# SavaRobotics/FoundationPose

Measured on AMD Instinct MI355X. Metric: pose-hypotheses/sec (render+refine+score), 252 hyp x 160x160, higher is better.
Workload: dtype f16

## Files before the change

foundationpose_amd/csrc/attn.hip:

```cpp
#include "common.h"
#include "device_util.h"
#include "pose_math.h"

#define AT_DH 128
#define AT_TP 416
#define AT_MAXT 400
#define FA_WAVES 7
#define FA_NSTAGE 3
#define FA_AHEAD 2
#define FA_DMA_PER_WAVE 5
#define FA_THREADS (FA_WAVES * 64)
#define FA_QB (FA_WAVES * 32)
#define FA_KB 64
#define FA_STAGE_HALFS (FA_KB * AT_DH * 2)
#define FA_QW_HALFS (32 * AT_DH)
#define FA_LDS_BYTES ((FA_NSTAGE * FA_STAGE_HALFS + FA_WAVES * FA_QW_HALFS) * 2)


typedef float f32x2 __attribute__((ext_vector_type(2)));
template <bool V> struct FaBool { static constexpr bool value = V; };

#ifdef HALO_STAMP
__device__ unsigned long long g_attn_stamps[1024 * 7 * 32];
extern "C" __attribute__((visibility("default"))) int fp_dbg_attn_stamps(unsigned long long *host) {
  return hipMemcpyFromSymbol(host, HIP_SYMBOL(g_attn_stamps), sizeof(g_attn_stamps)) == hipSuccess ? 0 : -1;
}
#define ASTAMP(i) do { if (blockIdx.x < 1024 && stamp_on) st[(i)] = __builtin_amdgcn_s_memtime(); } while (0)
#else
#define ASTAMP(i) do { } while (0)
#endif

__device__ __forceinline__ float fa_max3(float a, float b, float c) {
  float r;
  asm("v_max3_f32 %0, %1, %2, %3" : "=v"(r) : "v"(a), "v"(b), "v"(c));
  return r;
}

__global__ __launch_bounds__(FA_THREADS, 2) void attention_kernel(const f16 *__restrict__ qk, const f16 *__restrict__ vt, int T,
                                                                  f16 *__restrict__ out, int n_items) {
  extern __shared__ __attribute__((aligned(16))) f16 smem[];
  const int nqb = (T + FA_QB - 1) / FA_QB;
  const int tid = threadIdx.x, lane = tid & 63, wave = __builtin_amdgcn_readfirstlane(tid >> 6);
  const int lr = lane & 31, lh = lane >> 5;
  const int nkb = (T + FA_KB - 1) / FA_KB;
  const int G = gridDim.x;
  f16 *qlds = smem + FA_NSTAGE * FA_STAGE_HALFS + wave * FA_QW_HALFS;
#ifdef HALO_STAMP
  unsigned long long st[32];
#pragma unroll
  for (int i = 0; i < 32; ++i) st[i] = 0;
  bool stamp_on = true;
#endif
  ASTAMP(0);

  auto item_of = [&](int v, int &b, int &h, int &qb) __attribute__((always_inline)) {
    const int L = xcd_remap(v, n_items);
    qb = L % nqb;
    h = (L / nqb) & 3;
    b = L / (nqb * 4);
  };

  unsigned sx[FA_DMA_PER_WAVE], sadd[FA_DMA_PER_WAVE];
#pragma unroll
  for (int u = 0; u < FA_DMA_PER_WAVE; ++u) {
    int i = wave + u * FA_WAVES;
    if (i >= 32) i -= 32;
    if (i < 16) {
      const int c = i * 64 + lane, kl = c >> 4, chp = c & 15;
      sx[u] = kl;
      sadd[u] = ((chp ^ (kl & 15)) * 8) * 2;
    } else {
      const int c = (i - 16) * 64 + lane, d = c >> 3, chp = c & 7;
      sx[u] = (chp ^ ((d >> 1) & 7)) * 8;
      sadd[u] = d * AT_TP * 2;
    }
  }
  int s_v = blockIdx.x, s_kb = 0, s_slot = 0;
  const f16 *s_kbase, *s_vsrc;
  auto stage_bases = [&]() __attribute__((always_inline)) {
    int b, h, qb;
    item_of(s_v, b, h, qb);
    s_kbase = qk + (size_t)b * T * 1024 + 512 + h * AT_DH;
    s_vsrc = vt + ((size_t)b * 4 + h) * AT_DH * AT_TP;
  };
  stage_bases();
  auto stage_next = [&]() __attribute__((always_inline)) {
#pragma unroll
    for (int u = 0; u < FA_DMA_PER_WAVE; ++u) {
      int i = wave + u * FA_WAVES;
      if (i >= 32) i -= 32;
      const bool is_k = i < 16;
      const unsigned t = min((unsigned)(s_kb * FA_KB) + sx[u], is_k ? (unsigned)(T - 1) : 408u);
      const unsigned voff = t * (is_k ? 2048u : 2u) + sadd[u];
      glds16(is_k ? s_kbase : s_vsrc, voff, smem + s_slot * FA_STAGE_HALFS + i * 512);
    }
    s_slot = s_slot + 1 == FA_NSTAGE ? 0 : s_slot + 1;
    if (++s_kb == nkb) {
      s_kb = 0;
      s_v += G;
      if (s_v < n_items) stage_bases();
    }
  };
  const unsigned qrow = wave * 32 + lr;
  auto stage_q = [&](int v) __attribute__((always_inline)) {
    int b, h, qb;
    item_of(v, b, h, qb);
    const f16 *qbase = qk + ((size_t)b * T + qb * FA_QB) * 1024 + h * AT_DH;
    const unsigned voff = min(qrow, (unsigned)(T - 1 - qb * FA_QB)) * 2048u + lh * 16;
#pragma unroll
    for (int s = 0; s < 8; ++s) glds16(qbase + s * 16, voff, qlds + s * 512);
  };

  unsigned koffb[8], voffb[4];
#pragma unroll
  for (int s = 0; s < 8; ++s) koffb[s] = (lr * AT_DH + (((2 * s + lh) ^ (lr & 15)) * 8)) * 2;
#pragma unroll
  for (int s = 0; s < 4; ++s) voffb[s] = FA_KB * AT_DH * 2 + (lr * FA_KB + (((2 * s + lh) ^ ((lr >> 1) & 7)) * 8)) * 2;

  const float c2 = 0.08838834764831845f * 1.4426950408889634f;
  const f32x2 c2v = {c2, c2};

  int inflight = 0;
#pragma unroll
  for (int p = 0; p < FA_AHEAD; ++p)
    if (s_v < n_items) {
      stage_next();
      ++inflight;
    }
  stage_q((int)blockIdx.x);

  half8 qf[8];
  floatx16 oacc[4];
  float m_run, l_run;
  int c_slot = 0;
  int st_prev = 0;
  bool first = true;

  for (int v = blockIdx.x; v < n_items; v += G) {
    int b, h, qb;
    item_of(v, b, h, qb);
    const size_t rowbase = (size_t)b * T;
    const int q = qb * FA_QB + wave * 32 + lr;
    const bool wave_valid = qb * FA_QB + wave * 32 < T;
    const bool has_next = v + G < n_items;
#ifdef HALO_STAMP
    stamp_on = v == (int)blockIdx.x + G || n_items <= G;
#endif
    ASTAMP(1);
#pragma unroll
    for (int dt = 0; dt < 4; ++dt)
#pragma unroll
      for (int e = 0; e < 16; ++e) oacc[dt][e] = 0.f;
    m_run = -1.0e30f;
    l_run = 0.f;

    auto body = [&](const int kb, auto first_c, auto tail_c) __attribute__((always_inline)) {
      constexpr bool KB0 = decltype(first_c)::value;
      constexpr bool TAIL = decltype(tail_c)::value;
      int allowed = inflight > 1 ? 5 : 0;
      if (KB0) allowed = first ? 0 : (nkb == 1 ? st_prev : allowed + st_prev);
      else if (kb == 1 && has_next) allowed += 8;
      if (allowed == 0) wait_vm_lgkm<0>();
      else if (allowed == 5) wait_vm_lgkm<5>();
      else if (allowed == 8) wait_vm_lgkm<8>();
      else wait_vm_lgkm<13>();
      __builtin_amdgcn_s_barrier();
      __builtin_amdgcn_sched_barrier(0);
      ASTAMP(3 + 4 * kb);
      if (s_v < n_items) {
        stage_next();
        ++inflight;
      }
      if constexpr (KB0) {
#pragma unroll
        for (int s = 0; s < 8; ++s) qf[s] = *reinterpret_cast<const half8 *>(qlds + s * 512 + lane * 8);
      }
      const char *sb = reinterpret_cast<const char *>(smem) + c_slot * (FA_STAGE_HALFS * 2);
      floatx16 sacc[2];
#pragma unroll
      for (int sh = 0; sh < 2; ++sh) {
        half8 kf[2][4];
#pragma unroll
        for (int s = 0; s < 4; ++s)
#pragma unroll
          for (int kt = 0; kt < 2; ++kt) kf[kt][s] = *reinterpret_cast<const half8 *>(sb + koffb[sh * 4 + s] + kt * (32 * AT_DH * 2));
        __builtin_amdgcn_sched_barrier(0);
#pragma unroll
        for (int s = 0; s < 4; ++s)
#pragma unroll
          for (int kt = 0; kt < 2; ++kt) {
            if (sh == 0 && s == 0) {
              const floatx16 zero = {0.f, 0.f, 0.f, 0.f, 0.f, 0.f, 0.f, 0.f, 0.f, 0.f, 0.f, 0.f, 0.f, 0.f, 0.f, 0.f};
              sacc[kt] = __builtin_amdgcn_mfma_f32_32x32x16_f16(kf[kt][s], qf[0], zero, 0, 0, 0);
            } else {
              sacc[kt] = __builtin_amdgcn_mfma_f32_32x32x16_f16(kf[kt][s], qf[sh * 4 + s], sacc[kt], 0, 0, 0);
            }
          }
      }
      __builtin_amdgcn_sched_barrier(0);
      ASTAMP(4 + 4 * kb);
      if constexpr (KB0) {
        if (has_next) stage_q(v + G);
      }
      if constexpr (TAIL) {
#pragma unroll
        for (int kt = 0; kt < 2; ++kt)
#pragma unroll
          for (int r = 0; r < 16; ++r) {
            const int key = kb * FA_KB + kt * 32 + (r & 3) + 8 * (r >> 2) + 4 * lh;
            sacc[kt][r] = key < T ? sacc[kt][r] : -1.0e30f;
          }
      }
      float bm = fmaxf(sacc[0][15], sacc[1][15]);
      bm = fa_max3(bm, sacc[0][0], sacc[1][0]);
#pragma unroll
      for (int r = 1; r < 15; r += 2) bm = fa_max3(bm, sacc[0][r], sacc[0][r + 1]);
#pragma unroll
      for (int r = 1; r < 15; r += 2) bm = fa_max3(bm, sacc[1][r], sacc[1][r + 1]);
      bm = fmaxf(bm, __shfl_xor(bm, 32));
      const float m_new = fmaxf(m_run, bm);
      const float alpha = __builtin_amdgcn_exp2f((m_run - m_new) * c2);
      const float nmc = -m_new * c2;
      const f32x2 nmcv = {nmc, nmc};
      f32x2 ps2 = {0.f, 0.f};
#pragma unroll
      for (int kt = 0; kt < 2; ++kt)
#pragma unroll
        for (int r = 0; r < 16; r += 2) {
          const f32x2 sv = {sacc[kt][r], sacc[kt][r + 1]};
          const f32x2 ev = __builtin_elementwise_fma(sv, c2v, nmcv);
          const f32x2 e = {__builtin_amdgcn_exp2f(ev.x), __builtin_amdgcn_exp2f(ev.y)};
          sacc[kt][r] = e.x;
          sacc[kt][r + 1] = e.y;
          ps2 += e;
        }
      float ps = ps2.x + ps2.y;
      ps += __shfl_xor(ps, 32);
      l_run = l_run * alpha + ps;
      if (__builtin_amdgcn_ballot_w64(m_new != m_run) != 0) {
#pragma unroll
        for (int dt = 0; dt < 4; ++dt)
#pragma unroll
          for (int e = 0; e < 16; ++e) oacc[dt][e] *= alpha;
      }
      m_run = m_new;
      half8 pf[2][2];
#pragma unroll
      for (int kt = 0; kt < 2; ++kt)
#pragma unroll
        for (int s2 = 0; s2 < 2; ++s2)
#pragma unroll
          for (int j = 0; j < 8; ++j) pf[kt][s2][j] = (f16)sacc[kt][8 * s2 + j];
      __builtin_amdgcn_sched_barrier(0);
      ASTAMP(5 + 4 * kb);
#pragma unroll
      for (int kt = 0; kt < 2; ++kt) {
        half8 vf[2][4];
#pragma unroll
        for (int s2 = 0; s2 < 2; ++s2)
#pragma unroll
          for (int dt = 0; dt < 4; ++dt) vf[s2][dt] = *reinterpret_cast<const half8 *>(sb + voffb[kt * 2 + s2] + dt * (32 * FA_KB * 2));
        __builtin_amdgcn_sched_barrier(0);
#pragma unroll
        for (int s2 = 0; s2 < 2; ++s2)
#pragma unroll
          for (int dt = 0; dt < 4; ++dt) oacc[dt] = __builtin_amdgcn_mfma_f32_32x32x16_f16(vf[s2][dt], pf[kt][s2], oacc[dt], 0, 0, 0);
      }
      __builtin_amdgcn_sched_barrier(0);
      ASTAMP(6 + 4 * kb);
      c_slot = c_slot + 1 == FA_NSTAGE ? 0 : c_slot + 1;
      --inflight;
    };
    if (nkb == 1) {
      body(0, FaBool<true>{}, FaBool<true>{});
    } else {
      body(0, FaBool<true>{}, FaBool<false>{});
      for (int kb = 1; kb < nkb - 1; ++kb) body(kb, FaBool<false>{}, FaBool<false>{});
      body(nkb - 1, FaBool<false>{}, FaBool<true>{});
    }

    if (wave_valid) {
      const float inv = 1.f / l_run;
      f16 *orow = out + (rowbase + min(q, T - 1)) * 512 + h * AT_DH + lh * 8;
#pragma unroll
      for (int dt = 0; dt < 4; ++dt)
#pragma unroll
        for (int gq = 0; gq < 4; gq += 2) {
          half4 ha, hb;
#pragma unroll
          for (int j = 0; j < 4; ++j) ha[j] = (f16)(oacc[dt][gq * 4 + j] * inv), hb[j] = (f16)(oacc[dt][(gq + 1) * 4 + j] * inv);
          const uint2 ua = __builtin_bit_cast(uint2, ha), ub = __builtin_bit_cast(uint2, hb);
          const auto r0 = __builtin_amdgcn_permlane32_swap(ua.x, ub.x, false, false);
          const auto r1 = __builtin_amdgcn_permlane32_swap(ua.y, ub.y, false, false);
          const uint4 ov = {r0[0], r1[0], r0[1], r1[1]};
          if (q < T) *reinterpret_cast<uint4 *>(orow + dt * 32 + gq * 8) = ov;
        }
    }
    ASTAMP(2);
    st_prev = wave_valid ? 8 : 0;
    first = false;
  }
#ifdef HALO_STAMP
  if (blockIdx.x < 1024 && lane == 0) {
    st[31] = __builtin_amdgcn_s_memtime();
    unsigned long long *o = g_attn_stamps + ((size_t)blockIdx.x * 7 + wave) * 32;
#pragma unroll
    for (int i = 0; i < 32; ++i) o[i] = st[i];
  }
#endif
}

#define FS_WAVES 7
#define FS_KP 136
#define FS_VP 72
#define FS_AREA_BYTES (AT_DH * FS_VP * 2)
#define FS_LDS_BYTES (FS_WAVES * FS_AREA_BYTES + 2 * FS_WAVES * 32 * 4)
static_assert(64 * FS_KP * 2 <= FS_AREA_BYTES && AT_DH * 32 * 4 <= FS_AREA_BYTES, "attention_small: wave area");
__global__ __launch_bounds__(FS_WAVES * 64) void attention_small_kernel(const f16 *__restrict__ qk, const f16 *__restrict__ vt, int T, f16 *__restrict__ out) {
  extern __shared__ __attribute__((aligned(16))) char fs_lds[];
  float *fs_m = reinterpret_cast<float *>(fs_lds + FS_WAVES * FS_AREA_BYTES), *fs_l = fs_m + FS_WAVES * 32;
  const int tid = threadIdx.x, lane = tid & 63, w = __builtin_amdgcn_readfirstlane(tid >> 6), lr = lane & 31, lh = lane >> 5;
  const int nqt = (T + 31) >> 5, nkb = (T + 63) >> 6;
  const int qt = blockIdx.x % nqt, h = (blockIdx.x / nqt) & 3, b = blockIdx.x / (nqt * 4);
  const float c2 = 0.08838834764831845f * 1.4426950408889634f;
  f16 *area = reinterpret_cast<f16 *>(fs_lds + (size_t)w * FS_AREA_BYTES);
  if (w < nkb) {
    u32x4 kq[16], vq[16];
    {
      const f16 *kbase = qk + (size_t)b * T * 1024 + 512 + h * AT_DH;
#pragma unroll
      for (int u = 0; u < 16; ++u) {
        const int i = lane + 64 * u, key = min(w * 64 + (i >> 4), T - 1);
        kq[u] = *reinterpret_cast<const u32x4 *>(kbase + (size_t)key * 1024 + (i & 15) * 8);
      }
      const f16 *vbase = vt + ((size_t)b * 4 + h) * AT_DH * AT_TP;
#pragma unroll
      for (int u = 0; u < 16; ++u) {
        const int i = lane + 64 * u, col = min(w * 64 + (i & 7) * 8, 408);
        vq[u] = *reinterpret_cast<const u32x4 *>(vbase + (size_t)(i >> 3) * AT_TP + col);
      }
    }
    half8 qf[8];
    {
      const f16 *qrow = qk + ((size_t)b * T + min(qt * 32 + lr, T - 1)) * 1024 + h * AT_DH + lh * 8;
#pragma unroll
      for (int s = 0; s < 8; ++s) qf[s] = *reinterpret_cast<const half8 *>(qrow + s * 16);
    }
#pragma unroll
    for (int u = 0; u < 16; ++u) {
      const int i = lane + 64 * u;
      *reinterpret_cast<u32x4 *>(area + (i >> 4) * FS_KP + (i & 15) * 8) = kq[u];
    }
    wait_lgkm();
    half8 kf[2][8];
#pragma unroll
    for (int kt = 0; kt < 2; ++kt)
#pragma unroll
      for (int s = 0; s < 8; ++s) kf[kt][s] = *reinterpret_cast<const half8 *>(area + (kt * 32 + lr) * FS_KP + s * 16 + lh * 8);
    floatx16 sacc[2];
#pragma unroll
    for (int kt = 0; kt < 2; ++kt) {
#pragma unroll
      for (int e = 0; e < 16; ++e) sacc[kt][e] = 0.f;
#pragma unroll
      for (int s = 0; s < 8; ++s) sacc[kt] = __builtin_amdgcn_mfma_f32_32x32x16_f16(kf[kt][s], qf[s], sacc[kt], 0, 0, 0);
    }
#pragma unroll
    for (int kt = 0; kt < 2; ++kt)
#pragma unroll
      for (int r = 0; r < 16; ++r) {
        const int key = w * 64 + kt * 32 + (r & 3) + 8 * (r >> 2) + 4 * lh;
        sacc[kt][r] = key < T ? sacc[kt][r] : -1.0e30f;
      }
    float bm = fmaxf(sacc[0][0], sacc[1][0]);
#pragma unroll
    for (int r = 1; r < 16; ++r) bm = fmaxf(bm, fmaxf(sacc[0][r], sacc[1][r]));
    bm = fmaxf(bm, __shfl_xor(bm, 32));
    const float nmc = -bm * c2;
    float ps = 0.f;
#pragma unroll
    for (int kt = 0; kt < 2; ++kt)
#pragma unroll
      for (int r = 0; r < 16; ++r) {
        const float e = __builtin_amdgcn_exp2f(fmaf(sacc[kt][r], c2, nmc));
        sacc[kt][r] = e;
        ps += e;
      }
    ps += __shfl_xor(ps, 32);
    wait_lgkm();
#pragma unroll
    for (int u = 0; u < 16; ++u) {
      const int i = lane + 64 * u;
      *reinterpret_cast<u32x4 *>(area + (i >> 3) * FS_VP + (i & 7) * 8) = vq[u];
    }
    wait_lgkm();
    floatx16 oacc[4];
#pragma unroll
    for (int dt = 0; dt < 4; ++dt)
#pragma unroll
      for (int e = 0; e < 16; ++e) oacc[dt][e] = 0.f;
#pragma unroll
    for (int kt = 0; kt < 2; ++kt) {
      if (w * 64 + kt * 32 >= T) continue;
#pragma unroll
      for (int s2 = 0; s2 < 2; ++s2) {
        half8 pf;
#pragma unroll
        for (int j = 0; j < 8; ++j) pf[j] = (f16)sacc[kt][8 * s2 + j];
#pragma unroll
        for (int dt = 0; dt < 4; ++dt)
          oacc[dt] = __builtin_amdgcn_mfma_f32_32x32x16_f16(*reinterpret_cast<const half8 *>(area + (dt * 32 + lr) * FS_VP + kt * 32 + s2 * 16 + lh * 8), pf,
                                                            oacc[dt], 0, 0, 0);
      }
    }
    wait_lgkm();
    float *po = reinterpret_cast<float *>(area) + lr;
#pragma unroll
    for (int dt = 0; dt < 4; ++dt)
#pragma unroll
      for (int r = 0; r < 16; ++r) po[(dt * 32 + (r & 3) + 8 * (r >> 2) + 4 * lh) * 32] = oacc[dt][r];
    if (lh == 0) fs_m[w * 32 + lr] = bm, fs_l[w * 32 + lr] = ps;
  }
  __syncthreads();
  if (tid >= 256) return;
  const int ql = tid & 31, dg = tid >> 5, q = qt * 32 + ql;
  if (q >= T) return;
  float m = fs_m[ql];
  for (int k = 1; k < nkb; ++k) m = fmaxf(m, fs_m[k * 32 + ql]);
  float l = 0.f, o[16];
#pragma unroll
  for (int i = 0; i < 16; ++i) o[i] = 0.f;
  for (int k = 0; k < nkb; ++k) {
    const float sc = __builtin_amdgcn_exp2f((fs_m[k * 32 + ql] - m) * c2);
    l += fs_l[k * 32 + ql] * sc;
    const float *pk = reinterpret_cast<const float *>(fs_lds + (size_t)k * FS_AREA_BYTES) + dg * 16 * 32 + ql;
#pragma unroll
    for (int i = 0; i < 16; ++i) o[i] = fmaf(pk[i * 32], sc, o[i]);
  }
  const float inv = 1.f / l;
  half8 h0, h1;
#pragma unroll
  for (int i = 0; i < 8; ++i) h0[i] = (f16)(o[i] * inv), h1[i] = (f16)(o[8 + i] * inv);
  f16 *orow = out + ((size_t)b * T + q) * 512 + h * AT_DH + dg * 16;
  *reinterpret_cast<half8 *>(orow) = h0;
  *reinterpret_cast<half8 *>(orow + 8) = h1;
}

void attn_kernel_lds(std::vector<KernelLds> &v) {
  v.push_back({(const void *)attention_kernel, (int)FA_LDS_BYTES});
  v.push_back({(const void *)attention_small_kernel, (int)FS_LDS_BYTES});
}

int launch_attention(fp_ctx *ctx, const f16 *qk, const f16 *vt, int B, int T, f16 *out, hipStream_t s) {
  FP_REQUIRE(T > 0 && T <= AT_MAXT, "attention: T=%d must be in [1,%d]", T, AT_MAXT);
  if (B == 0) return FP_OK;
  if (attn_form(B, pass_knobs()) == ATTN_SMALL) {
    ProfScope ps(ctx, s, "attention", 4.0 * B * 4 * (double)T * T * AT_DH);
    hipLaunchKernelGGL(attention_small_kernel, dim3(((T + 31) / 32) * 4 * B), dim3(FS_WAVES * 64), FS_LDS_BYTES, s, qk, vt, T, out);
    FP_CHECK_HIP(hipGetLastError());
    return FP_OK;
  }
  const int n_items = ((T + FA_QB - 1) / FA_QB) * 4 * B;
  const int grid = n_items < ctx->num_cu ? n_items : ctx->num_cu;
  ProfScope ps(ctx, s, "attention", 4.0 * B * 4 * (double)T * T * AT_DH);
  hipLaunchKernelGGL(attention_kernel, dim3(grid), dim3(FA_THREADS), FA_LDS_BYTES, s, qk, vt, T, out, n_items);
  FP_CHECK_HIP(hipGetLastError());
  return FP_OK;
}

#define MH_MAXPARTS 32
template <int NH>
__device__ __forceinline__ void mean_head_rows(float (*meanv)[512], int b, const float *const *partial, int nparts, const float *const *gam,
                                               const float *const *bet, int T) {
  const int f = threadIdx.x;
  float v[NH][MH_MAXPARTS];
#pragma unroll
  for (int h = 0; h < NH; ++h)
#pragma unroll
    for (int u = 0; u < MH_MAXPARTS; ++u) v[h][u] = partial[h][((size_t)b * nparts + min(u, nparts - 1)) * 512 + f];
#pragma unroll
  for (int h = 0; h < NH; ++h) {
    float m = 0.f;
#pragma unroll
    for (int u = 0; u < MH_MAXPARTS; ++u)
      if (u < nparts) m += v[h][u];
    meanv[h][f] = m * (1.f / (float)T) * gam[h][f] + bet[h][f];
  }
}
__device__ __forceinline__ float mean_head_out(const float *meanv, const float *__restrict__ hw, const float *__restrict__ hb, int o, int lane) {
  float s = 0.f;
#pragma unroll
  for (int i = 0; i < 8; ++i) s += meanv[lane * 8 + i] * hw[(size_t)o * 512 + lane * 8 + i];
  s = wave_sum(s);
  return s + hb[o];
}

__global__ __launch_bounds__(512) void mean_head_kernel(const float *__restrict__ partial, int nparts, const float *__restrict__ gam,
                                                        const float *__restrict__ bet, int T, const float *__restrict__ hw,
                                                        const float *__restrict__ hb, int out_dim, float *__restrict__ out) {
  __shared__ float meanv[1][512];
  const int b = blockIdx.x, wave = threadIdx.x >> 6, lane = threadIdx.x & 63;
  const float *p1[1] = {partial}, *g1[1] = {gam}, *b1[1] = {bet};
  mean_head_rows<1>(meanv, b, p1, nparts, g1, b1, T);
  __syncthreads();
  for (int o = wave; o < out_dim; o += 8) {
    const float r = mean_head_out(meanv[0], hw, hb, o, lane);
    if (lane == 0) out[(size_t)b * out_dim + o] = r;
  }
}

template <bool OBJS>
__global__ __launch_bounds__(512) void refine_tail_kernel(RefineTailArgs a) {
  __shared__ float meanv[2][512], delta[2][8];
  const int b = blockIdx.x, wave = threadIdx.x >> 6, lane = threadIdx.x & 63;
  mean_head_rows<2>(meanv, b, a.partial, a.nparts, a.gam, a.bet, a.T);
  __syncthreads();
  for (int o = wave; o < 3 + a.rot_dim; o += 8) {
    const int h = o >= 3, oh = h ? o - 3 : o;
    const float r = mean_head_out(meanv[h], a.hw[h], a.hb[h], oh, lane);
    if (lane == 0) {
      (h ? a.rot + (size_t)b * a.rot_dim : a.trans + (size_t)b * 3)[oh] = r;
      delta[h][oh] = r;
    }
  }
  __syncthreads();
  if (threadIdx.x != 0) return;
  DeepimArgs dp;
  dp.tf = a.tf;
  dp.resize = a.resize;
  for (int i = 0; i < 9; ++i) dp.K[i] = a.K[i];
  if constexpr (OBJS) {
    pose_update_one(b, a.poses, delta[0], delta[1], a.rot_dim, a.trans_tanh, a.tn0, a.tn1, a.tn2, a.rot_normalizer, a.obj.trans_scale[b], dp, a.poses);
    if (a.next_window) {
      CropWindowK w = a.win;
      w.radius = a.obj.radius[b];
      crop_window_tf_one(b, a.poses, w, a.tf, a.bbox);
    }
    const float *p = a.poses + (size_t)b * 16;
    if (float *c = a.obj.centered[b]) pose_of_mesh_one(p, a.obj.cneg[b], c);
    if (float *o = a.obj.pose_out[b])
#pragma unroll
      for (int i = 0; i < 16; ++i) o[i] = p[i];
  } else {
    pose_update_one(b, a.poses, delta[0], delta[1], a.rot_dim, a.trans_tanh, a.tn0, a.tn1, a.tn2, a.rot_normalizer, a.trans_scale, dp, a.poses);
    if (a.next_window) crop_window_tf_one(b, a.poses, a.win, a.tf, a.bbox);
    if (a.centered) pose_of_mesh_one(a.poses + (size_t)b * 16, a.cneg, a.centered + (size_t)b * 16);
  }
}

int launch_refine_tail(const RefineTailArgs &a, int N, hipStream_t s) {
  FP_REQUIRE(a.rot_dim == 3 || a.rot_dim == 6, "refine tail: rot_dim must be 3 or 6");
  FP_REQUIRE(a.nparts >= 1 && a.nparts <= MH_MAXPARTS, "refine tail: %d partial rows per hypothesis (at most %d)", a.nparts, MH_MAXPARTS);
  FP_REQUIRE(a.obj.n == 0 || (a.obj.n == N && N <= FP_TRACK_MAX_OBJECTS), "refine tail: %d hypotheses for %d objects", N, a.obj.n);
  if (N == 0) return FP_OK;
  if (a.obj.n) hipLaunchKernelGGL(refine_tail_kernel<true>, dim3(N), dim3(512), 0, s, a);
  else hipLaunchKernelGGL(refine_tail_kernel<false>, dim3(N), dim3(512), 0, s, a);
  FP_CHECK_HIP(hipGetLastError());
  return FP_OK;
}

int launch_mean_head(const float *partial, int nparts, const float *g, const float *b, int Bn, int T, const float *hw, const float *hb,
                     int out_dim, float *out, hipStream_t s) {
  FP_REQUIRE(nparts >= 1 && nparts <= MH_MAXPARTS, "mean_head: %d partial rows per hypothesis (at most %d)", nparts, MH_MAXPARTS);
  if (Bn == 0) return FP_OK;
  hipLaunchKernelGGL(mean_head_kernel, dim3(Bn), dim3(512), 0, s, partial, nparts, g, b, T, hw, hb, out_dim, out);
  FP_CHECK_HIP(hipGetLastError());
  return FP_OK;
}

__global__ void pose_update_kernel(const float *__restrict__ poseA, const float *__restrict__ trans, const float *__restrict__ rot,
                                   int N, int rot_dim, int trans_tanh, float tn0, float tn1, float tn2, float rot_normalizer,
                                   float trans_scale, DeepimArgs dp, float *__restrict__ outp) {
  const int b = blockIdx.x * blockDim.x + threadIdx.x;
  if (b >= N) return;
  pose_update_one(b, poseA, trans + (size_t)b * 3, rot + (size_t)b * rot_dim, rot_dim, trans_tanh, tn0, tn1, tn2, rot_normalizer, trans_scale, dp, outp);
}

int launch_pose_update(const float *poseA, const float *trans, const float *rot, int N, int rot_dim, int trans_tanh, float tn0,
                       float tn1, float tn2, float rot_normalizer, float trans_scale, float *out, hipStream_t s, const float *tf,
                       const double *K, float resize) {
  FP_REQUIRE(rot_dim == 3 || rot_dim == 6, "pose_update: rot_dim must be 3 or 6");
  FP_REQUIRE(trans_tanh >= 0 && trans_tanh <= 2, "pose_update: trans mode %d unknown (0 raw, 1 tanh, 2 deepim)", trans_tanh);
  FP_REQUIRE(trans_tanh != 2 || (tf && K), "pose_update: trans_rep='deepim' needs the crop transforms and K");
  if (N == 0) return FP_OK;
  DeepimArgs dp;
  dp.tf = tf;
  dp.resize = resize;
  for (int i = 0; i < 9; ++i) dp.K[i] = K ? (float)K[i] : 0.f;
  hipLaunchKernelGGL(pose_update_kernel, dim3((N + 63) / 64), dim3(64), 0, s, poseA, trans, rot, N, rot_dim, trans_tanh, tn0, tn1, tn2,
                     rot_normalizer, trans_scale, dp, out);
  FP_CHECK_HIP(hipGetLastError());
  return FP_OK;
}
```

foundationpose_amd/csrc/net.hip:

```cpp
#include "common.h"
#include "device_util.h"

#include <algorithm>
#include <cmath>
#include <cstdlib>
#include <memory>

struct ConvW {
  f16 *w = nullptr;
  f16 *wpk = nullptr;
  f16 *wsm = nullptr;
  f16 *wfr = nullptr;
  float *bias = nullptr;
  int Cin = 0, Cout = 0, K = 1, Kpad = 0, stride = 1;
};

struct LinP {
  f16 *w = nullptr;
  float *bias = nullptr;
};

struct HeadW {
  LinP q, k, v, out, ff1, ff2;
  float *ln1g = nullptr, *ln1b = nullptr, *ln2g = nullptr, *ln2b = nullptr, *hw = nullptr, *hb = nullptr;
  int out_dim = 0;
};

struct LinF32 {
  float *w = nullptr, *b = nullptr, *wt = nullptr;
  int N = 0, K = 0;
};

struct fp_net {
  int kind = 0, use_bn = 1;
  ConvW trunk[15];
  float *pe = nullptr;
  HeadW heads[2];
  LinP att_q, att_k, att_v;
  LinF32 att_out;
  float *tail_wqk_t = nullptr, *tail_bqk = nullptr;
  double *tail_u = nullptr, *tail_c = nullptr, tail_b_eff = 0.0;
  std::vector<void *> allocs;
};

const PassKnobs &pass_knobs() {
  static const PassKnobs knobs = [] {
    PassKnobs k;
    k.chunk = (int)fp_env_int("FP_CHUNK", k.chunk);
    k.trunk_min = (int)fp_env_int("FP_TRUNK_MIN", k.trunk_min);
    k.trunk_streams = (int)fp_env_int("FP_TRUNK_STREAMS", k.trunk_streams);
    k.one_chain = fp_env_int("FP_ONE_CHAIN", 0) != 0;
    k.no_shared_b = fp_env_set("FP_NO_SHARED_B");
    k.tail_split = fp_env_set("FP_TAIL_SPLIT");
    k.qkv_small = (int)fp_env_int("FP_QKV_SMALL", k.qkv_small);
    k.qkv64 = fp_env_set("FP_QKV64");
    k.attn_small = (int)fp_env_int("FP_ATTN_SMALL", k.attn_small);
    k.headmlp64 = fp_env_set("FP_HEADMLP64");
    k.heads_serial = fp_env_set("FP_HEADS_SERIAL");
    k.front_fused = fp_env_int("FP_FRONT_FUSED", 1) != 0;
    return k;
  }();
  return knobs;
}

namespace {

struct SD {
  std::map<std::string, const fp_tensor *> m;
  const fp_tensor *get(const std::string &k) const {
    auto it = m.find(k);
    return it == m.end() ? nullptr : it->second;
  }
};

int need(const SD &sd, const std::string &k, int ndim, std::initializer_list<int64_t> shape, const fp_tensor **out) {
  const fp_tensor *t = sd.get(k);
  if (!t) {
    fp_set_error("state_dict: missing key '%s'", k.c_str());
    return FP_EKEY;
  }
  if (t->ndim != ndim) {
    fp_set_error("state_dict: '%s' has ndim %d, expected %d", k.c_str(), t->ndim, ndim);
    return FP_EKEY;
  }
  int i = 0;
  for (int64_t s : shape) {
    if (s >= 0 && t->shape[i] != s) {
      fp_set_error("state_dict: '%s' dim %d is %lld, expected %lld", k.c_str(), i, (long long)t->shape[i], (long long)s);
      return FP_EKEY;
    }
    ++i;
  }
  *out = t;
  return FP_OK;
}

template <typename T>
int upload(fp_net *net, const std::vector<T> &h, T **d) {
  void *p = nullptr;
  FP_CHECK_HIP(hipMalloc(&p, h.size() * sizeof(T)));
  net->allocs.push_back(p);
  FP_CHECK_HIP(hipMemcpy(p, h.data(), h.size() * sizeof(T), hipMemcpyHostToDevice));
  *d = (T *)p;
  return FP_OK;
}

int make_conv(fp_net *net, const SD &sd, const std::string &wkey, const std::string &bnkey, bool use_bn, int stride, ConvW *out) {
  const fp_tensor *w, *b;
  FP_TRY(need(sd, wkey + ".weight", 4, {-1, -1, -1, -1}, &w));
  const int Cout = (int)w->shape[0], Cin = (int)w->shape[1], K = (int)w->shape[2];
  FP_REQUIRE(w->shape[3] == K, "conv '%s' is not square", wkey.c_str());
  FP_TRY(need(sd, wkey + ".bias", 1, {Cout}, &b));
  std::vector<float> scale(Cout, 1.f), shift(Cout, 0.f);
  if (use_bn) {
    const fp_tensor *g, *be, *mu, *var;
    FP_TRY(need(sd, bnkey + ".weight", 1, {Cout}, &g));
    FP_TRY(need(sd, bnkey + ".bias", 1, {Cout}, &be));
    FP_TRY(need(sd, bnkey + ".running_mean", 1, {Cout}, &mu));
    FP_TRY(need(sd, bnkey + ".running_var", 1, {Cout}, &var));
    for (int c = 0; c < Cout; ++c) {
      scale[c] = g->data[c] / std::sqrt(var->data[c] + 1e-5f);
      shift[c] = be->data[c] - mu->data[c] * scale[c];
    }
  }
  const int CinP = (Cin < 8) ? 8 : Cin;
  FP_REQUIRE(CinP == 8 || CinP % 32 == 0, "conv '%s': Cin=%d unsupported", wkey.c_str(), Cin);
  const int Kpad = conv_kpad(K, K, CinP);
  std::vector<f16> hw((size_t)Cout * Kpad, (f16)0.f);
  std::vector<float> hb(Cout);
  for (int co = 0; co < Cout; ++co) {
    for (int ci = 0; ci < Cin; ++ci)
      for (int ky = 0; ky < K; ++ky)
        for (int kx = 0; kx < K; ++kx)
          hw[(size_t)co * Kpad + (ky * K + kx) * CinP + ci] = (f16)(w->data[(((size_t)co * Cin + ci) * K + ky) * K + kx] * scale[co]);
    hb[co] = b->data[co] * scale[co] + shift[co];
  }
  out->Cin = CinP;
  out->Cout = Cout;
  out->K = K;
  out->Kpad = Kpad;
  out->stride = stride;
  FP_TRY(upload(net, hw, &out->w));
  FP_TRY(upload(net, hb, &out->bias));
  const unsigned packings = conv_packings(CinP, Cout, K, stride, Kpad);
  for (const unsigned pk : {packings & (CONV_OFFER_S2 | CONV_OFFER_S1B), packings & CONV_OFFER_SMALL}) {
    if (!pk) continue;
    void *d = nullptr;
    FP_CHECK_HIP(hipMalloc(&d, conv_packed_halfs(pk, Cout, CinP) * sizeof(f16)));
    net->allocs.push_back(d);
    (pk == CONV_OFFER_SMALL ? out->wsm : out->wpk) = (f16 *)d;
    FP_TRY(conv_pack_weights(pk, out->w, Cout, CinP, Kpad, (f16 *)d, nullptr));
    FP_CHECK_HIP(hipStreamSynchronize(nullptr));
  }
  if (K == 7 && CinP == 8 && Cout == 64 && stride == 2) {
    void *d = nullptr;
    FP_CHECK_HIP(hipMalloc(&d, front_packed_stem_halfs() * sizeof(f16)));
    net->allocs.push_back(d);
    out->wfr = (f16 *)d;
    FP_TRY(front_pack_stem(out->w, Kpad, out->wfr, nullptr));
    FP_CHECK_HIP(hipStreamSynchronize(nullptr));
  }
  return FP_OK;
}

void pack_tok_weights(const float *w, f16 *out) {
  for (int wave = 0; wave < 4; ++wave)
    for (int k16 = 0; k16 < 32; ++k16)
      for (int i = 0; i < 4; ++i)
        for (int lane = 0; lane < 64; ++lane) {
          const int lr = lane & 31, lh = lane >> 5;
          const float *src = w + (size_t)(wave * 128 + i * 32 + lr) * 512 + k16 * 16 + lh * 8;
          f16 *dst = out + ((((size_t)wave * 32 + k16) * 4 + i) * 64 + lane) * 8;
          for (int e = 0; e < 8; ++e) dst[e] = (f16)src[e];
        }
}

int make_linear(fp_net *net, const SD &sd, const std::string &wkey, const std::string &bkey, int r0, LinP *out) {
  const fp_tensor *w, *b;
  FP_TRY(need(sd, wkey, 2, {-1, 512}, &w));
  FP_TRY(need(sd, bkey, 1, {w->shape[0]}, &b));
  FP_REQUIRE(r0 + 512 <= w->shape[0], "linear '%s': rows out of range", wkey.c_str());
  std::vector<f16> hw((size_t)512 * 512);
  std::vector<float> hb(512);
  pack_tok_weights(w->data + (size_t)r0 * 512, hw.data());
  for (int n = 0; n < 512; ++n) hb[n] = b->data[r0 + n];
  FP_TRY(upload(net, hw, &out->w));
  FP_TRY(upload(net, hb, &out->bias));
  return FP_OK;
}

int make_vec(fp_net *net, const SD &sd, const std::string &key, int n, float **out) {
  const fp_tensor *t = sd.get(key);
  if (!t) {
    fp_set_error("state_dict: missing key '%s'", key.c_str());
    return FP_EKEY;
  }
  int64_t tot = 1;
  for (int i = 0; i < t->ndim; ++i) tot *= t->shape[i];
  FP_REQUIRE(tot == n, "state_dict: '%s' has %lld elements, expected %d", key.c_str(), (long long)tot, n);
  std::vector<float> h(t->data, t->data + n);
  return upload(net, h, out);
}

int make_linf32(fp_net *net, const SD &sd, const std::string &wkey, const std::string &bkey, int N, int K, LinF32 *out) {
  out->N = N;
  out->K = K;
  FP_TRY(make_vec(net, sd, wkey, N * K, &out->w));
  FP_TRY(make_vec(net, sd, bkey, N, &out->b));
  const fp_tensor *t = sd.get(wkey);
  std::vector<float> tr((size_t)N * K);
  for (int n = 0; n < N; ++n)
    for (int k = 0; k < K; ++k) tr[(size_t)k * N + n] = t->data[(size_t)n * K + k];
  return upload(net, tr, &out->wt);
}

int make_score_tail(fp_net *net, const SD &sd) {
  const fp_tensor *wi, *bi, *wo, *bo, *lw, *lb;
  FP_TRY(need(sd, "att_cross.in_proj_weight", 2, {1536, 512}, &wi));
  FP_TRY(need(sd, "att_cross.in_proj_bias", 1, {1536}, &bi));
  FP_TRY(need(sd, "att_cross.out_proj.weight", 2, {512, 512}, &wo));
  FP_TRY(need(sd, "att_cross.out_proj.bias", 1, {512}, &bo));
  FP_TRY(need(sd, "linear.weight", 2, {1, 512}, &lw));
  FP_TRY(need(sd, "linear.bias", 1, {1}, &lb));
  std::vector<float> wt((size_t)512 * 1024), bqk(1024);
  for (int n = 0; n < 1024; ++n) {
    bqk[n] = bi->data[n];
    for (int k = 0; k < 512; ++k) wt[(size_t)k * 1024 + n] = wi->data[(size_t)n * 512 + k];
  }
  std::vector<double> weff(512, 0.0), u((size_t)4 * 512, 0.0), c(4, 0.0);
  double beff = (double)lb->data[0];
  for (int n = 0; n < 512; ++n) {
    const double l = (double)lw->data[n];
    beff += l * (double)bo->data[n];
    for (int k = 0; k < 512; ++k) weff[k] += l * (double)wo->data[(size_t)n * 512 + k];
  }
  for (int h = 0; h < 4; ++h)
    for (int d = 0; d < 128; ++d) {
      const double w = weff[h * 128 + d];
      const float *vr = wi->data + (size_t)(1024 + h * 128 + d) * 512;
      c[h] += w * (double)bi->data[1024 + h * 128 + d];
      for (int k = 0; k < 512; ++k) u[(size_t)h * 512 + k] += w * (double)vr[k];
    }
  net->tail_b_eff = beff;
  FP_TRY(upload(net, wt, &net->tail_wqk_t));
  FP_TRY(upload(net, bqk, &net->tail_bqk));
  FP_TRY(upload(net, u, &net->tail_u));
  FP_TRY(upload(net, c, &net->tail_c));
  return FP_OK;
}

int make_trunk(fp_net *net, const SD &sd, const std::string &eA, const std::string &eAB, bool bn) {
  auto cbr = [&](const std::string &pre, int stride, ConvW *o) { return make_conv(net, sd, pre + ".net.0", pre + ".net.1", bn, stride, o); };
  auto res = [&](const std::string &pre, ConvW *o1, ConvW *o2) {
    FP_TRY(make_conv(net, sd, pre + ".conv1", pre + ".bn1", bn, 1, o1));
    return make_conv(net, sd, pre + ".conv2", pre + ".bn2", bn, 1, o2);
  };
  ConvW *t = net->trunk;
  FP_TRY(cbr(eA + ".0", 2, &t[0]));
  FP_TRY(cbr(eA + ".1", 2, &t[1]));
  FP_TRY(res(eA + ".2", &t[2], &t[3]));
  FP_TRY(res(eA + ".3", &t[4], &t[5]));
  FP_TRY(res(eAB + ".0", &t[6], &t[7]));
  FP_TRY(res(eAB + ".1", &t[8], &t[9]));
  FP_TRY(cbr(eAB + ".2", 2, &t[10]));
  FP_TRY(res(eAB + ".3", &t[11], &t[12]));
  FP_TRY(res(eAB + ".4", &t[13], &t[14]));
  FP_REQUIRE(t[0].Cin == 8 && t[0].Cout == 64 && t[0].K == 7 && t[1].Cout == 128 && t[6].Cin == 256 && t[10].Cout == 512,
             "trunk: unexpected layer shapes (c_in must be <= 8 -> padded to 8)");
  FP_TRY(make_vec(net, sd, "pos_embed.pe", 400 * 512, &net->pe));
  return FP_OK;
}

}

extern "C" int fp_net_create(fp_ctx *ctx, int kind, const fp_tensor *tensors, int n_tensors, int use_bn, fp_net **out) {
  FP_REQUIRE(ctx && tensors && out, "fp_net_create: null argument");
  FP_REQUIRE(kind == FP_NET_REFINE || kind == FP_NET_SCORE, "fp_net_create: kind must be FP_NET_REFINE or FP_NET_SCORE");
  FP_CHECK_HIP(hipSetDevice(ctx->device));
  SD sd;
  for (int i = 0; i < n_tensors; ++i) sd.m[tensors[i].name] = &tensors[i];
  std::unique_ptr<fp_net> net(new fp_net);
  net->kind = kind;
  net->use_bn = use_bn;
  int rc = FP_OK;
  auto run = [&]() -> int {
    if (kind == FP_NET_REFINE) {
      FP_TRY(make_trunk(net.get(), sd, "encodeA", "encodeAB", use_bn));
      const char *names[2] = {"trans_head", "rot_head"};
      for (int h = 0; h < 2; ++h) {
        HeadW &H = net->heads[h];
        std::string p = std::string(names[h]) + ".0";
        FP_TRY(make_linear(net.get(), sd, p + ".self_attn.in_proj_weight", p + ".self_attn.in_proj_bias", 0, &H.q));
        FP_TRY(make_linear(net.get(), sd, p + ".self_attn.in_proj_weight", p + ".self_attn.in_proj_bias", 512, &H.k));
        FP_TRY(make_linear(net.get(), sd, p + ".self_attn.in_proj_weight", p + ".self_attn.in_proj_bias", 1024, &H.v));
        FP_TRY(make_linear(net.get(), sd, p + ".self_attn.out_proj.weight", p + ".self_attn.out_proj.bias", 0, &H.out));
        FP_TRY(make_linear(net.get(), sd, p + ".linear1.weight", p + ".linear1.bias", 0, &H.ff1));
        FP_TRY(make_linear(net.get(), sd, p + ".linear2.weight", p + ".linear2.bias", 0, &H.ff2));
        FP_TRY(make_vec(net.get(), sd, p + ".norm1.weight", 512, &H.ln1g));
        FP_TRY(make_vec(net.get(), sd, p + ".norm1.bias", 512, &H.ln1b));
        FP_TRY(make_vec(net.get(), sd, p + ".norm2.weight", 512, &H.ln2g));
        FP_TRY(make_vec(net.get(), sd, p + ".norm2.bias", 512, &H.ln2b));
        const fp_tensor *hw;
        FP_TRY(need(sd, std::string(names[h]) + ".1.weight", 2, {-1, 512}, &hw));
        H.out_dim = (int)hw->shape[0];
        FP_REQUIRE(H.out_dim >= 1 && H.out_dim <= 6, "head '%s': out_dim %d unsupported", names[h], H.out_dim);
        FP_TRY(make_vec(net.get(), sd, std::string(names[h]) + ".1.weight", H.out_dim * 512, &H.hw));
        FP_TRY(make_vec(net.get(), sd, std::string(names[h]) + ".1.bias", H.out_dim, &H.hb));
      }
    } else {
      FP_TRY(make_trunk(net.get(), sd, "encoderA", "encoderAB", use_bn));
      FP_TRY(make_linear(net.get(), sd, "att.in_proj_weight", "att.in_proj_bias", 0, &net->att_q));
      FP_TRY(make_linear(net.get(), sd, "att.in_proj_weight", "att.in_proj_bias", 512, &net->att_k));
      FP_TRY(make_linear(net.get(), sd, "att.in_proj_weight", "att.in_proj_bias", 1024, &net->att_v));
      FP_TRY(make_linf32(net.get(), sd, "att.out_proj.weight", "att.out_proj.bias", 512, 512, &net->att_out));
      FP_TRY(make_score_tail(net.get(), sd));
    }
    return FP_OK;
  };
  rc = run();
  if (rc != FP_OK) {
    for (void *p : net->allocs) (void)hipFree(p);
    return rc;
  }
  *out = net.release();
  return FP_OK;
}

extern "C" int fp_net_destroy(fp_net *net) {
  if (!net) return FP_OK;
  for (void *p : net->allocs) (void)hipFree(p);
  delete net;
  return FP_OK;
}

extern "C" int fp_net_rot_dim(const fp_net *net) { return (net && net->kind == FP_NET_REFINE) ? net->heads[1].out_dim : 0; }

namespace {

struct Conv2dCall {
  const f16 *in;
  int Nimg, H, W;
  const ConvW *cw;
  const f16 *res = nullptr;
  int relu = 1;
  void *out = nullptr;
  int out_mode = 0;
  int out_ld = 0, split_m = 0x7fffffff, coff_hi = 0;
  const float *post_add = nullptr;
  int post_period = 1;
  int tokens = 400;
};

int run_conv(fp_ctx *ctx, const Conv2dCall &c, hipStream_t s, float *splitk_scratch = nullptr, int hyp = 0) {
  const ConvW &w = *c.cw;
  ConvArgs a = conv_args(c.in, c.Nimg, c.H, c.W, w.Cin, w.w, w.bias, w.Cout, w.K, w.K, w.stride, (w.K - 1) / 2, w.Kpad, c.out);
  a.wpk = w.wpk, a.wsm = w.wsm, a.splitk = splitk_scratch, a.hyp = hyp;
  a.res = c.res, a.relu = c.relu, a.out_mode = c.out_mode;
  if (c.out_ld) a.out_ld = c.out_ld;
  a.split_m = c.split_m, a.coff_hi = c.coff_hi;
  a.post_add = c.post_add, a.post_period = c.post_period, a.tokens = c.tokens;
  return launch_conv(ctx, a, s);
}
// ... 414 lines not shown
```

foundationpose_amd/csrc/pass_plan.h:

```cpp
#pragma once
#include <limits.h>

#include "conv_plan.h"

struct PassKnobs {
  int chunk = 0;
  int trunk_min = 48;
  int trunk_streams = 2;
  bool one_chain = false;
  bool no_shared_b = false;
  bool tail_split = false;
  int qkv_small = 2;
  bool qkv64 = false;
  int attn_small = 2;
  bool headmlp64 = false;
  bool heads_serial = false;
  bool front_fused = true;
};
const PassKnobs &pass_knobs();

enum PassKind { PASS_REFINE = 0, PASS_SCORE = 1 };
enum AttnForm { ATTN_SMALL, ATTN_PERSISTENT };
enum HeadMlpForm { HEAD_MLP_64, HEAD_MLP_128, HEAD_MLP_NONE };
enum QkvForm { QKV_SMALL, QKV_TOK128, QKV_PAIR64 };

#define PASS_SIDE_STREAMS 8
#define PASS_SHARED_B_MAX_OBJECTS 8
#define PASS_FLAG_SHARED_TRANSLATION 1u

inline AttnForm attn_form(int images, const PassKnobs &k) { return images <= k.attn_small ? ATTN_SMALL : ATTN_PERSISTENT; }

inline HeadMlpForm head_mlp_form(int M, const PassKnobs &k) { return k.headmlp64 || M <= 1600 ? HEAD_MLP_64 : HEAD_MLP_128; }

inline QkvForm qkv_form(int hyp, int images, const PassKnobs &k) {
  if (hyp > 0 && hyp <= k.qkv_small) return QKV_SMALL;
  if (hyp > 0 && k.qkv64 && images > k.qkv_small) return QKV_PAIR64;
  return QKV_TOK128;
}

inline bool front_fused(int images, int hyp, bool splitk, int num_cu, const PassKnobs &k, const ConvKnobs &ck) {
  if (!k.front_fused || images <= 0) return false;
  ConvArgs st = conv_args(nullptr, images, 160, 160, 8, nullptr, nullptr, 64, 7, 7, 2, 3, conv_kpad(7, 7, 8), nullptr);
  ConvArgs dn = conv_args(nullptr, images, 80, 80, 64, nullptr, nullptr, 128, 3, 3, 2, 1, conv_kpad(3, 3, 64), nullptr);
  st.relu = dn.relu = 1, st.hyp = dn.hyp = hyp;
  const unsigned sk = splitk ? CONV_OFFER_SPLITK : 0u;
  return conv_plan(st, num_cu, sk, ck).form == CONV_STEM && conv_plan(dn, num_cu, CONV_OFFER_SMALL | CONV_OFFER_S2 | sk, ck).form == CONV_IGEMM2;
}

inline int trunk_split_min(const PassKnobs &k) { return k.trunk_streams < 2 ? INT_MAX : k.trunk_min; }
inline int trunk_parts(int n, const PassKnobs &k, int n_side_streams) {
  if (n < trunk_split_min(k)) return 1;
  const int by_size = n / 32 > 2 ? n / 32 : 2;
  const int cap = k.trunk_streams < n_side_streams ? k.trunk_streams : n_side_streams;
  return cap < by_size ? cap : by_size;
}

inline bool net_offers_splitk(int n) { return n <= CONV_NET_SPLITK_MAX_HYP; }

inline int hyp_chunk(int n_total, const PassKnobs &k) { return k.chunk <= 0 || k.chunk > n_total ? n_total : k.chunk; }

struct ForwardPlan {
  int n;
  int trunk_parts;
  QkvForm qkv;
  AttnForm attn;
  HeadMlpForm head_mlp;
  int head_streams;
};

inline ForwardPlan forward_plan(int kind, int n, const PassKnobs &k, int n_side_streams = PASS_SIDE_STREAMS) {
  ForwardPlan p;
  p.n = n;
  p.trunk_parts = trunk_parts(n, k, n_side_streams);
  p.qkv = qkv_form(n, n, k);
  p.attn = attn_form(n, k);
  p.head_mlp = kind == PASS_REFINE ? head_mlp_form(n * 400, k) : HEAD_MLP_NONE;
  p.head_streams = kind == PASS_REFINE ? (k.heads_serial ? 1 : 2) : 0;
  return p;
}

struct TrunkPart {
  int start, n, conv_hyp;
  bool splitk;
};
inline TrunkPart trunk_part(const ForwardPlan &p, int i) {
  const int a0 = (int)((long long)p.n * i / p.trunk_parts), a1 = (int)((long long)p.n * (i + 1) / p.trunk_parts);
  return TrunkPart{a0, a1 - a0, a1 - a0, net_offers_splitk(a1 - a0)};
}

struct PassPlan {
  int chunk;
  bool fork_sides;
  bool side_chains;
  bool shared_b;
  bool fused_tail;
};

inline PassPlan pass_plan(int kind, int n_total, int n_runs, int n_live, unsigned flags, const PassKnobs &k) {
  PassPlan p;
  p.chunk = hyp_chunk(n_total, k);
  const bool whole = p.chunk == n_total, refine_run = kind == PASS_REFINE && n_runs == 1 && whole;
  p.fork_sides = n_runs == 1 && n_total < trunk_split_min(k) && !k.one_chain;
  p.side_chains = p.fork_sides && whole;
  p.shared_b = refine_run && (flags & PASS_FLAG_SHARED_TRANSLATION) && !k.no_shared_b && n_live <= PASS_SHARED_B_MAX_OBJECTS;
  p.fused_tail = refine_run && !k.tail_split;
  return p;
}

inline const char *attn_form_name(AttnForm f) { return f == ATTN_SMALL ? "attn-small" : "attn-persistent"; }
inline const char *head_mlp_form_name(HeadMlpForm f) { return f == HEAD_MLP_64 ? "mlp64" : f == HEAD_MLP_128 ? "mlp128" : "none"; }
inline const char *qkv_form_name(QkvForm f) { return f == QKV_SMALL ? "qkv-small" : f == QKV_TOK128 ? "qkv128" : "qkv64-pair"; }
```

Measured before the change: 7466.

## Add lean attention variant skipping padded key slices and dead query waves

Templates the flash-attention kernel on a LEAN flag. The lean variant trims the final key block's QK and PV MFMAs to the 16-key slices actually covered by T. It skips all compute for waves whose query rows fall past T while keeping barrier and staging participation. It also seeds the accumulator with the first PV MFMA instead of zeroing and rescaling. It is enabled by default via an env knob, at the cost of extra template instantiations and more complex tail masking logic.

```diff
diff --git a/foundationpose_amd/csrc/attn.hip b/foundationpose_amd/csrc/attn.hip
--- a/foundationpose_amd/csrc/attn.hip
+++ b/foundationpose_amd/csrc/attn.hip
@@ -19,6 +19,7 @@
 
 typedef float f32x2 __attribute__((ext_vector_type(2)));
 template <bool V> struct FaBool { static constexpr bool value = V; };
+template <int N> struct FaInt { static constexpr int value = N; };
 
 #ifdef HALO_STAMP
 __device__ unsigned long long g_attn_stamps[1024 * 7 * 32];
@@ -36,13 +37,15 @@
   return r;
 }
 
-__global__ __launch_bounds__(FA_THREADS, 2) void attention_kernel(const f16 *__restrict__ qk, const f16 *__restrict__ vt, int T,
+template <bool LEAN>
+__global__ __launch_bounds__(FA_THREADS, 2) void attention_kernel(const f16 *__restrict__ qk, const f16 *__restrict__ vt, int T, int tail,
                                                                   f16 *__restrict__ out, int n_items) {
   extern __shared__ __attribute__((aligned(16))) f16 smem[];
   const int nqb = (T + FA_QB - 1) / FA_QB;
   const int tid = threadIdx.x, lane = tid & 63, wave = __builtin_amdgcn_readfirstlane(tid >> 6);
   const int lr = lane & 31, lh = lane >> 5;
   const int nkb = (T + FA_KB - 1) / FA_KB;
+  const int nks = (tail + 15) >> 4;
   const int G = gridDim.x;
   f16 *qlds = smem + FA_NSTAGE * FA_STAGE_HALFS + wave * FA_QW_HALFS;
 #ifdef HALO_STAMP
@@ -147,16 +150,17 @@
     stamp_on = v == (int)blockIdx.x + G || n_items <= G;
 #endif
     ASTAMP(1);
-#pragma unroll
-    for (int dt = 0; dt < 4; ++dt)
-#pragma unroll
-      for (int e = 0; e < 16; ++e) oacc[dt][e] = 0.f;
+    if constexpr (!LEAN) {
+#pragma unroll
+      for (int dt = 0; dt < 4; ++dt)
+#pragma unroll
+        for (int e = 0; e < 16; ++e) oacc[dt][e] = 0.f;
+    }
     m_run = -1.0e30f;
     l_run = 0.f;
 
-    auto body = [&](const int kb, auto first_c, auto tail_c) __attribute__((always_inline)) {
+    auto block_sync = [&](const int kb, auto first_c) __attribute__((always_inline)) {
       constexpr bool KB0 = decltype(first_c)::value;
-      constexpr bool TAIL = decltype(tail_c)::value;
       int allowed = inflight > 1 ? 5 : 0;
       if (KB0) allowed = first ? 0 : (nkb == 1 ? st_prev : allowed + st_prev);
       else if (kb == 1 && has_next) allowed += 8;
@@ -171,24 +175,42 @@
         stage_next();
         ++inflight;
       }
+    };
+    auto next_q = [&](auto first_c) __attribute__((always_inline)) {
+      if constexpr (decltype(first_c)::value) {
+        if (has_next) stage_q(v + G);
+      }
+    };
+    auto block_done = [&]() __attribute__((always_inline)) {
+      c_slot = c_slot + 1 == FA_NSTAGE ? 0 : c_slot + 1;
+      --inflight;
+    };
+    auto body = [&](const int kb, auto first_c, auto tail_c, auto nks_c) __attribute__((always_inline)) {
+      constexpr bool KB0 = decltype(first_c)::value;
+      constexpr bool TAIL = decltype(tail_c)::value;
+      constexpr int NKS = decltype(nks_c)::value;
+      constexpr int NKT = (NKS + 1) / 2, NR = 8 * NKS;
+      static_assert(NKS >= 1 && NKS <= 4 && (NKS == 4 || (LEAN && TAIL)), "attention: only a lean tail block is short");
+#define FA_S(f) sacc[(f) >> 4][(f) & 15]
+      block_sync(kb, first_c);
       if constexpr (KB0) {
 #pragma unroll
         for (int s = 0; s < 8; ++s) qf[s] = *reinterpret_cast<const half8 *>(qlds + s * 512 + lane * 8);
       }
       const char *sb = reinterpret_cast<const char *>(smem) + c_slot * (FA_STAGE_HALFS * 2);
-      floatx16 sacc[2];
+      floatx16 sacc[NKT];
 #pragma unroll
       for (int sh = 0; sh < 2; ++sh) {
-        half8 kf[2][4];
+        half8 kf[NKT][4];
 #pragma unroll
         for (int s = 0; s < 4; ++s)
 #pragma unroll
-          for (int kt = 0; kt < 2; ++kt) kf[kt][s] = *reinterpret_cast<const half8 *>(sb + koffb[sh * 4 + s] + kt * (32 * AT_DH * 2));
+          for (int kt = 0; kt < NKT; ++kt) kf[kt][s] = *reinterpret_cast<const half8 *>(sb + koffb[sh * 4 + s] + kt * (32 * AT_DH * 2));
         __builtin_amdgcn_sched_barrier(0);
 #pragma unroll
         for (int s = 0; s < 4; ++s)
 #pragma unroll
-          for (int kt = 0; kt < 2; ++kt) {
+          for (int kt = 0; kt < NKT; ++kt) {
             if (sh == 0 && s == 0) {
               const floatx16 zero = {0.f, 0.f, 0.f, 0.f, 0.f, 0.f, 0.f, 0.f, 0.f, 0.f, 0.f, 0.f, 0.f, 0.f, 0.f, 0.f};
               sacc[kt] = __builtin_amdgcn_mfma_f32_32x32x16_f16(kf[kt][s], qf[0], zero, 0, 0, 0);
@@ -199,10 +221,8 @@
       }
       __builtin_amdgcn_sched_barrier(0);
       ASTAMP(4 + 4 * kb);
-      if constexpr (KB0) {
-        if (has_next) stage_q(v + G);
-      }
-      if constexpr (TAIL) {
+      next_q(first_c);
+      if constexpr (TAIL && !LEAN) {
 #pragma unroll
         for (int kt = 0; kt < 2; ++kt)
 #pragma unroll
@@ -211,12 +231,42 @@
             sacc[kt][r] = key < T ? sacc[kt][r] : -1.0e30f;
           }
       }
-      float bm = fmaxf(sacc[0][15], sacc[1][15]);
-      bm = fa_max3(bm, sacc[0][0], sacc[1][0]);
-#pragma unroll
-      for (int r = 1; r < 15; r += 2) bm = fa_max3(bm, sacc[0][r], sacc[0][r + 1]);
-#pragma unroll
-      for (int r = 1; r < 15; r += 2) bm = fa_max3(bm, sacc[1][r], sacc[1][r + 1]);
+      if constexpr (TAIL && LEAN) {
+        constexpr int F0 = 8 * (NKS - 1);
+        const int rem = tail - 16 * (NKS - 1);
+        if (rem <= 8) {
+#pragma unroll
+          for (int j = 0; j < 4; ++j) FA_S(F0 + 4 + j) = -1.0e30f;
+          if (rem < 8) {
+#pragma unroll
+            for (int j = 0; j < 4; ++j) FA_S(F0 + j) = 4 * lh + j < rem ? FA_S(F0 + j) : -1.0e30f;
+          }
+        } else if (rem < 16) {
+#pragma unroll
+          for (int j = 0; j < 4; ++j) FA_S(F0 + 4 + j) = 8 + 4 * lh + j < rem ? FA_S(F0 + 4 + j) : -1.0e30f;
+        }
+      }
+      float bm;
+      if constexpr (NKS == 4) {
+        bm = fmaxf(sacc[0][15], sacc[1][15]);
+        bm = fa_max3(bm, sacc[0][0], sacc[1][0]);
+#pragma unroll
+        for (int r = 1; r < 15; r += 2) bm = fa_max3(bm, sacc[0][r], sacc[0][r + 1]);
+#pragma unroll
+        for (int r = 1; r < 15; r += 2) bm = fa_max3(bm, sacc[1][r], sacc[1][r + 1]);
+      } else {
+        constexpr int F1 = NKT == 2 ? 16 : 1;
+        bm = fmaxf(FA_S(0), FA_S(F1));
+        float pend = 0.f;
+        bool have = false;
+#pragma unroll
+        for (int f = 1; f < NR; ++f) {
+          if (f == F1) continue;
+          if (have) bm = fa_max3(bm, pend, FA_S(f));
+          else pend = FA_S(f);
+          have = !have;
+        }
+      }
       bm = fmaxf(bm, __shfl_xor(bm, 32));
       const float m_new = fmaxf(m_run, bm);
       const float alpha = __builtin_amdgcn_exp2f((m_run - m_new) * c2);
@@ -224,59 +274,90 @@
       const f32x2 nmcv = {nmc, nmc};
       f32x2 ps2 = {0.f, 0.f};
 #pragma unroll
-      for (int kt = 0; kt < 2; ++kt)
-#pragma unroll
-        for (int r = 0; r < 16; r += 2) {
-          const f32x2 sv = {sacc[kt][r], sacc[kt][r + 1]};
-          const f32x2 ev = __builtin_elementwise_fma(sv, c2v, nmcv);
-          const f32x2 e = {__builtin_amdgcn_exp2f(ev.x), __builtin_amdgcn_exp2f(ev.y)};
-          sacc[kt][r] = e.x;
-          sacc[kt][r + 1] = e.y;
-          ps2 += e;
-        }
+      for (int f = 0; f < NR; f += 2) {
+        const f32x2 sv = {FA_S(f), FA_S(f + 1)};
+        const f32x2 ev = __builtin_elementwise_fma(sv, c2v, nmcv);
+        const f32x2 e = {__builtin_amdgcn_exp2f(ev.x), __builtin_amdgcn_exp2f(ev.y)};
+        FA_S(f) = e.x;
+        FA_S(f + 1) = e.y;
+        ps2 += e;
+      }
       float ps = ps2.x + ps2.y;
       ps += __shfl_xor(ps, 32);
       l_run = l_run * alpha + ps;
-      if (__builtin_amdgcn_ballot_w64(m_new != m_run) != 0) {
-#pragma unroll
-        for (int dt = 0; dt < 4; ++dt)
-#pragma unroll
-          for (int e = 0; e < 16; ++e) oacc[dt][e] *= alpha;
+      if constexpr (!(LEAN && KB0)) {
+        if (__builtin_amdgcn_ballot_w64(m_new != m_run) != 0) {
+#pragma unroll
+          for (int dt = 0; dt < 4; ++dt)
+#pragma unroll
+            for (int e = 0; e < 16; ++e) oacc[dt][e] *= alpha;
+        }
       }
       m_run = m_new;
-      half8 pf[2][2];
-#pragma unroll
-      for (int kt = 0; kt < 2; ++kt)
-#pragma unroll
-        for (int s2 = 0; s2 < 2; ++s2)
-#pragma unroll
-          for (int j = 0; j < 8; ++j) pf[kt][s2][j] = (f16)sacc[kt][8 * s2 + j];
+      half8 pf[NKS];
+#pragma unroll
+      for (int ks = 0; ks < NKS; ++ks)
+#pragma unroll
+        for (int j = 0; j < 8; ++j) pf[ks][j] = (f16)FA_S(8 * ks + j);
       __builtin_amdgcn_sched_barrier(0);
       ASTAMP(5 + 4 * kb);
 #pragma unroll
-      for (int kt = 0; kt < 2; ++kt) {
+      for (int kt = 0; kt < NKT; ++kt) {
+        const int n2 = NKS - 2 * kt < 2 ? NKS - 2 * kt : 2;
         half8 vf[2][4];
 #pragma unroll
         for (int s2 = 0; s2 < 2; ++s2)
 #pragma unroll
-          for (int dt = 0; dt < 4; ++dt) vf[s2][dt] = *reinterpret_cast<const half8 *>(sb + voffb[kt * 2 + s2] + dt * (32 * FA_KB * 2));
+          for (int dt = 0; dt < 4; ++dt)
+            if (s2 < n2) vf[s2][dt] = *reinterpret_cast<const half8 *>(sb + voffb[kt * 2 + s2] + dt * (32 * FA_KB * 2));
         __builtin_amdgcn_sched_barrier(0);
 #pragma unroll
         for (int s2 = 0; s2 < 2; ++s2)
 #pragma unroll
-          for (int dt = 0; dt < 4; ++dt) oacc[dt] = __builtin_amdgcn_mfma_f32_32x32x16_f16(vf[s2][dt], pf[kt][s2], oacc[dt], 0, 0, 0);
-      }
+          for (int dt = 0; dt < 4; ++dt) {
+            if (s2 >= n2) continue;
+            if (LEAN && KB0 && kt == 0 && s2 == 0) {
+              const floatx16 zero = {0.f, 0.f, 0.f, 0.f, 0.f, 0.f, 0.f, 0.f, 0.f, 0.f, 0.f, 0.f, 0.f, 0.f, 0.f, 0.f};
+              oacc[dt] = __builtin_amdgcn_mfma_f32_32x32x16_f16(vf[s2][dt], pf[0], zero, 0, 0, 0);
+            } else {
+              oacc[dt] = __builtin_amdgcn_mfma_f32_32x32x16_f16(vf[s2][dt], pf[kt * 2 + s2], oacc[dt], 0, 0, 0);
+            }
+          }
+      }
+#undef FA_S
       __builtin_amdgcn_sched_barrier(0);
       ASTAMP(6 + 4 * kb);
-      c_slot = c_slot + 1 == FA_NSTAGE ? 0 : c_slot + 1;
-      --inflight;
+      block_done();
     };
-    if (nkb == 1) {
-      body(0, FaBool<true>{}, FaBool<true>{});
+    auto dead_body = [&](const int kb, auto first_c) __attribute__((always_inline)) {
+      block_sync(kb, first_c);
+      next_q(first_c);
+      ASTAMP(4 + 4 * kb);
+      ASTAMP(5 + 4 * kb);
+      ASTAMP(6 + 4 * kb);
+      block_done();
+    };
+    auto tail_body = [&](const int kb, auto first_c) __attribute__((always_inline)) {
+      if constexpr (LEAN) {
+        switch (nks) {
+          case 1: body(kb, first_c, FaBool<true>{}, FaInt<1>{}); break;
+          case 2: body(kb, first_c, FaBool<true>{}, FaInt<2>{}); break;
+          case 3: body(kb, first_c, FaBool<true>{}, FaInt<3>{}); break;
+          default: body(kb, first_c, FaBool<true>{}, FaInt<4>{}); break;
+        }
+      } else {
+        body(kb, first_c, FaBool<true>{}, FaInt<4>{});
+      }
+    };
+    if (LEAN && !wave_valid) {
+      dead_body(0, FaBool<true>{});
+      for (int kb = 1; kb < nkb; ++kb) dead_body(kb, FaBool<false>{});
+    } else if (nkb == 1) {
+      tail_body(0, FaBool<true>{});
     } else {
-      body(0, FaBool<true>{}, FaBool<false>{});
-      for (int kb = 1; kb < nkb - 1; ++kb) body(kb, FaBool<false>{}, FaBool<false>{});
-      body(nkb - 1, FaBool<false>{}, FaBool<true>{});
+      body(0, FaBool<true>{}, FaBool<false>{}, FaInt<4>{});
+      for (int kb = 1; kb < nkb - 1; ++kb) body(kb, FaBool<false>{}, FaBool<false>{}, FaInt<4>{});
+      tail_body(nkb - 1, FaBool<false>{});
     }
 
     if (wave_valid) {
@@ -447,7 +528,8 @@
 }
 
 void attn_kernel_lds(std::vector<KernelLds> &v) {
-  v.push_back({(const void *)attention_kernel, (int)FA_LDS_BYTES});
+  v.push_back({(const void *)attention_kernel<true>, (int)FA_LDS_BYTES});
+  v.push_back({(const void *)attention_kernel<false>, (int)FA_LDS_BYTES});
   v.push_back({(const void *)attention_small_kernel, (int)FS_LDS_BYTES});
 }
 
@@ -463,7 +545,9 @@
   const int n_items = ((T + FA_QB - 1) / FA_QB) * 4 * B;
   const int grid = n_items < ctx->num_cu ? n_items : ctx->num_cu;
   ProfScope ps(ctx, s, "attention", 4.0 * B * 4 * (double)T * T * AT_DH);
-  hipLaunchKernelGGL(attention_kernel, dim3(grid), dim3(FA_THREADS), FA_LDS_BYTES, s, qk, vt, T, out, n_items);
+  const int tail = T - FA_KB * ((T + FA_KB - 1) / FA_KB - 1);
+  if (pass_knobs().attn_lean) hipLaunchKernelGGL(attention_kernel<true>, dim3(grid), dim3(FA_THREADS), FA_LDS_BYTES, s, qk, vt, T, tail, out, n_items);
+  else hipLaunchKernelGGL(attention_kernel<false>, dim3(grid), dim3(FA_THREADS), FA_LDS_BYTES, s, qk, vt, T, tail, out, n_items);
   FP_CHECK_HIP(hipGetLastError());
   return FP_OK;
 }
diff --git a/foundationpose_amd/csrc/net.hip b/foundationpose_amd/csrc/net.hip
--- a/foundationpose_amd/csrc/net.hip
+++ b/foundationpose_amd/csrc/net.hip
@@ -58,6 +58,7 @@
     k.headmlp64 = fp_env_set("FP_HEADMLP64");
     k.heads_serial = fp_env_set("FP_HEADS_SERIAL");
     k.front_fused = fp_env_int("FP_FRONT_FUSED", 1) != 0;
+    k.attn_lean = fp_env_int("FP_ATTN_LEAN", 1) != 0;
     return k;
   }();
   return knobs;
diff --git a/foundationpose_amd/csrc/pass_plan.h b/foundationpose_amd/csrc/pass_plan.h
--- a/foundationpose_amd/csrc/pass_plan.h
+++ b/foundationpose_amd/csrc/pass_plan.h
@@ -16,6 +16,7 @@
   bool headmlp64 = false;
   bool heads_serial = false;
   bool front_fused = true;
+  bool attn_lean = true;
 };
 const PassKnobs &pass_knobs();
 
```

Measured after the change: 7489, median of 6. No clear change (+0.3%).
